# AnnaUshnova/tinyrenderder

Hardware: AMD Instinct MI355X
Metric: triangles/sec (+ Mpixels/sec) at 4096x4096; achieved HBM GB/s vs peak (higher is better)
Workload: dtype f64

## Files before the change

tinyrenderder_amd/csrc/kernels_bin.hip:

```cpp
#include <hip/hip_runtime.h>
#include <algorithm>
#include "trgl_device.h"
#include "launch.h"
#include "device_util.h"

namespace {

__device__ __forceinline__ double dmin3(double a, double b, double c) { double m = a; if (b < m) m = b; if (c < m) m = c; return m; }
__device__ __forceinline__ double dmax3(double a, double b, double c) { double m = a; if (m < b) m = b; if (m < c) m = c; return m; }
using trgl_dev::dot4; using trgl_dev::wave_incl_scan; using trgl_dev::block_excl_scan;

__device__ __forceinline__ int wave_min_i(int v) {
    for (int o = 32; o; o >>= 1) { int t = __shfl_xor(v, o); v = t < v ? t : v; }
    return v;
}
__device__ __forceinline__ int wave_max_i(int v) {
    for (int o = 32; o; o >>= 1) { int t = __shfl_xor(v, o); v = t > v ? t : v; }
    return v;
}

__device__ __forceinline__ uint32_t tile_block_mask(uint32_t tx, uint32_t ty, uint32_t qx0, uint32_t qy0, uint32_t qx1, uint32_t qy1) {
    const uint32_t c0 = qx0 > 4 * tx ? qx0 - 4 * tx : 0u, c1 = qx1 < 4 * tx + 3 ? qx1 - 4 * tx : 3u;
    const uint32_t r0 = qy0 > 4 * ty ? qy0 - 4 * ty : 0u, r1 = qy1 < 4 * ty + 3 ? qy1 - 4 * ty : 3u;
    return (((2u << c1) - (1u << c0)) & 0xfu) * 0x1111u & ((0xffffu >> (12 - 4 * r1)) & (0xffffu << (4 * r0)));
// ... 1 lines not shown
template <class Put>
__device__ __forceinline__ void block_pairs(const FrameParams& fp, int tiles_x, uint32_t i, uint32_t c, uint2 tb, uint32_t o, Put put) {
    constexpr uint32_t SMALL = 8;
    if (c && c <= SMALL) {
        const uint32_t qx0 = tb.x & 0x1fff, qy0 = (tb.x >> 16) & 0x1fff, qx1 = tb.y & 0x1fff, qy1 = (tb.y >> 16) & 0x1fff;
        const uint32_t iz = i | ((((tb.x >> 13) & 7u) | (((tb.y >> 13) & 7u) << 3) | ((tb.y >> 29) << 6)) << 25);
        const uint32_t tx0 = qx0 >> 2, ty0 = qy0 >> 2, tx1 = qx1 >> 2;
        uint32_t tx = tx0, row = 0;
        uint32_t ty = fp.il_tiles ? (uint32_t)il_nth_owned_from(fp, (int)ty0, 0) : ty0;
        for (uint32_t k = 0; k < c; ++k) {
            put(o + k, ty * tiles_x + tx, iz, tile_block_mask(tx, ty, qx0, qy0, qx1, qy1));
            if (++tx > tx1) { tx = tx0; ++row; ty = fp.il_tiles ? (uint32_t)il_nth_owned_from(fp, (int)ty0, (int)row) : ty0 + row; }
        }
    }
    unsigned long long big = __ballot(c > SMALL);
    const int lane = threadIdx.x & 63;
    while (big) {
        int src = __ffsll((long long)big) - 1;
        big &= big - 1;
        uint32_t cc = __shfl(c, src), oo = __shfl(o, src), ii = __shfl(i, src);
        uint32_t bx = __shfl(tb.x, src), by = __shfl(tb.y, src);
        const uint32_t qx0 = bx & 0x1fff, qy0 = (bx >> 16) & 0x1fff, qx1 = by & 0x1fff, qy1 = (by >> 16) & 0x1fff;
        ii |= (((bx >> 13) & 7u) | (((by >> 13) & 7u) << 3) | ((by >> 29) << 6)) << 25;
        uint32_t tx0 = qx0 >> 2, ty0 = qy0 >> 2, tx1 = qx1 >> 2;
        uint32_t wdt = tx1 - tx0 + 1;
        for (uint32_t k = lane; k < cc; k += 64) {
            uint32_t ty = fp.il_tiles ? (uint32_t)il_nth_owned_from(fp, (int)ty0, (int)(k / wdt)) : ty0 + k / wdt, tx = tx0 + k % wdt;
            put(oo + k, ty * tiles_x + tx, ii, tile_block_mask(tx, ty, qx0, qy0, qx1, qy1));
        }
    }
}

constexpr uint32_t SEG_MAX = 4096, SEG_MAX_GROUP = 16;

constexpr int SETUP_THREADS = 256;

__global__ __launch_bounds__(SETUP_THREADS) void k_setup(FrameParams fp, DrawDesc d, DrawDesc* __restrict__ draws_out, int draw_idx,
                                                         TriRec* __restrict__ recs, TriW* __restrict__ recs_w, uint32_t* __restrict__ cnt,
                                                         uint2* __restrict__ tilebox, DevStats* __restrict__ stats,
                                                         uint32_t* __restrict__ blk_sums, uint32_t blk_base,
                                                         uint32_t* __restrict__ seg_k, uint32_t* __restrict__ seg_v, uint32_t seg_S) {
    __shared__ __attribute__((aligned(16))) double s_buf[SETUP_THREADS * 16];
    if (blockIdx.x == 0 && threadIdx.x == 0) draws_out[draw_idx] = d;
    const uint32_t b0 = blockIdx.x * SETUP_THREADS;
    const uint32_t nb = min((uint32_t)SETUP_THREADS, d.n - b0);
    const uint32_t tid = threadIdx.x;
    const uint32_t i = b0 + tid;
    const bool in_range = tid < nb;

    const double* src = d.clip + (size_t)b0 * 12;
    if ((reinterpret_cast<uintptr_t>(src) & 15) == 0) {
        const double2* s2 = reinterpret_cast<const double2*>(src);
        double2* l2 = reinterpret_cast<double2*>(s_buf);
        typedef double f64x2 __attribute__((ext_vector_type(2)));
        for (uint32_t k = tid; k < nb * 6; k += SETUP_THREADS)
            *reinterpret_cast<f64x2*>(&l2[k]) = __builtin_nontemporal_load(reinterpret_cast<const f64x2*>(&s2[k]));
    } else {
        for (uint32_t k = tid; k < nb * 12; k += SETUP_THREADS) s_buf[k] = src[k];
    }
    __syncthreads();
    double v[12];
#pragma unroll
    for (int k = 0; k < 12; ++k) v[k] = in_range ? s_buf[tid * 12 + k] : 0.0;
    __syncthreads();

    int bx0 = INT_MAX, by0 = INT_MAX, bx1 = INT_MIN, by1 = INT_MIN;
    uint32_t ntiles = 0;
    bool large = false;
    uint2 tb = make_uint2(0, 0);
    TriRec r;
    {
        uint4* z4 = reinterpret_cast<uint4*>(&r);
#pragma unroll
        for (int k = 0; k < 8; ++k) z4[k] = make_uint4(0, 0, 0, 0);
// ... 97 lines not shown
        uint4* l4 = reinterpret_cast<uint4*>(s_buf);
        const uint4* r4 = reinterpret_cast<const uint4*>(&r);
#pragma unroll
        for (int c = 0; c < 8; ++c) l4[tid * 8 + (c ^ (tid & 7))] = r4[c];
        const unsigned long long keep = __ballot(ntiles != 0);
        __builtin_amdgcn_wave_barrier();
        uint4* dst = reinterpret_cast<uint4*>(recs + d.first + b0 + wbase);
#pragma unroll
        for (int it = 0; it < 8; ++it) {
            const uint32_t k = lane + 64u * it, t = k >> 3, c = k & 7;
            if ((keep >> t) & 1ull) {
                typedef uint32_t u32x4 __attribute__((ext_vector_type(4)));
                __builtin_nontemporal_store(*reinterpret_cast<const u32x4*>(&l4[(wbase + t) * 8 + (c ^ (t & 7))]), reinterpret_cast<u32x4*>(&dst[k]));
            }
        }
    }
    {
        const unsigned long long lit = __ballot(ntiles != 0 && r.ruz == 0.0);
        if (lit && lane == 0) atomicAdd(&stats->literal_tris, (unsigned long long)__popcll(lit));
        const unsigned long long lrg = __ballot(large);
        if (lrg && lane == 0) atomicAdd(&stats->large_tris, (unsigned long long)__popcll(lrg));
    }
    int wx0 = wave_min_i(bx0), wy0 = wave_min_i(by0), wx1 = wave_max_i(bx1), wy1 = wave_max_i(by1);
    if ((threadIdx.x & 63) == 0 && wx0 != INT_MAX) {
        if (wx0 < __builtin_nontemporal_load(&stats->min_x)) atomicMin(&stats->min_x, wx0);
        if (wy0 < __builtin_nontemporal_load(&stats->min_y)) atomicMin(&stats->min_y, wy0);
        if (wx1 > __builtin_nontemporal_load(&stats->max_x)) atomicMax(&stats->max_x, wx1);
        if (wy1 > __builtin_nontemporal_load(&stats->max_y)) atomicMax(&stats->max_y, wy1);
    }
    uint32_t tot;
    const uint32_t off = block_excl_scan(ntiles, reinterpret_cast<uint32_t*>(s_buf), &tot);
    if (tid == 0) blk_sums[blk_base + blockIdx.x] = tot;
    if (seg_S && tot && tot <= seg_S) {
        __syncthreads();
        uint32_t* const s_k = reinterpret_cast<uint32_t*>(s_buf);
        uint32_t* const s_v = s_k + SEG_MAX;
        block_pairs(fp, fp.tiles_x, d.first + i, ntiles, tb, off, [&](uint32_t j, uint32_t key, uint32_t iz, uint32_t m) { s_k[j] = key | (m << 16); s_v[j] = iz; });
        __syncthreads();
        uint4* const kq = reinterpret_cast<uint4*>(seg_k + (size_t)(blk_base + blockIdx.x) * seg_S);
        uint4* const vq = reinterpret_cast<uint4*>(seg_v + (size_t)(blk_base + blockIdx.x) * seg_S);
        for (uint32_t q = tid; 4 * q < tot; q += SETUP_THREADS) {
            kq[q] = *reinterpret_cast<const uint4*>(s_k + 4 * q);
            vq[q] = *reinterpret_cast<const uint4*>(s_v + 4 * q);
        }
    }
}

constexpr int EXPAND_CHUNK = 16;

constexpr int SPINE_THREADS = 1024;
__global__ __launch_bounds__(SPINE_THREADS) void k_chunk_spine(const uint32_t* __restrict__ blk_sums, uint32_t nblk,
                                                               uint32_t* __restrict__ chunk_off,
                                                               unsigned long long* __restrict__ total64, unsigned long long* __restrict__ host_copy,
                                                               uint4* __restrict__ bounds16, uint32_t n_half16,
                                                               uint32_t seg_S, uint32_t seg_G, uint32_t seg_chunk,
                                                               uint32_t* __restrict__ seg_flag, uint32_t* __restrict__ seg_flag_host) {
    __shared__ unsigned long long s_wave[SPINE_THREADS / 64];
    int seg_bad = seg_S == 0;
    if (seg_S && seg_G != EXPAND_CHUNK) {
        for (uint32_t g = threadIdx.x; (uint64_t)g * seg_G < nblk; g += SPINE_THREADS) {
            uint32_t t[EXPAND_CHUNK];
#pragma unroll
            for (uint32_t k = 0; k < EXPAND_CHUNK; ++k) { const uint32_t q = g * seg_G + k; t[k] = (k < seg_G && q < nblk) ? blk_sums[q] : 0u; }
            unsigned long long sum = 0;
#pragma unroll
            for (uint32_t k = 0; k < EXPAND_CHUNK; ++k) sum += t[k];
            seg_bad |= sum > seg_chunk;
        }
    }
    const uint32_t blk_max = seg_S ? seg_S : ~0u;
    const unsigned long long grp_max = (seg_S && seg_G == EXPAND_CHUNK) ? seg_chunk : ~0ull;
    for (uint32_t k = threadIdx.x; k < 2 * n_half16; k += SPINE_THREADS) bounds16[k] = k < n_half16 ? make_uint4(~0u, ~0u, ~0u, ~0u) : make_uint4(0, 0, 0, 0);
    const uint32_t nchunks = (nblk + EXPAND_CHUNK - 1) / EXPAND_CHUNK;
    const int lane = threadIdx.x & 63, w = threadIdx.x >> 6;
    unsigned long long running = 0;
    for (uint32_t start = 0; start < nchunks; start += SPINE_THREADS) {
        const uint32_t c = start + threadIdx.x;
        unsigned long long v = 0;
        if (c < nchunks) {
            const uint32_t q0 = c * EXPAND_CHUNK;
            if (q0 + EXPAND_CHUNK <= nblk) {
                const uint4* p4 = reinterpret_cast<const uint4*>(blk_sums + q0);
#pragma unroll
                for (int k = 0; k < EXPAND_CHUNK / 4; ++k) {
                    const uint4 t = p4[k]; v += (unsigned long long)t.x + t.y + t.z + t.w;
                    seg_bad |= max(max(t.x, t.y), max(t.z, t.w)) > blk_max;
                }
            } else {
                for (uint32_t q = q0; q < nblk; ++q) { const uint32_t t = blk_sums[q]; v += t; seg_bad |= t > blk_max; }
// ... 70 lines not shown
                    if (j >= sh && j < end) { kq[j] = s_k[j]; vq[j] = s_v[j]; if (WIDE) mq[j] = s_m[j]; }
            }
        }
    }
}

constexpr int RADIX_ROUNDS = 16;
constexpr int RADIX_WAVE_CHUNK = RADIX_ROUNDS * 64;
constexpr uint32_t RADIX_BIG_CAP = 4u << 20;
constexpr int RADIX_MAX_BITS = 8;

__global__ __launch_bounds__(256) void k_radix_hist(const uint32_t* __restrict__ keys, const unsigned long long* __restrict__ pairs_total,
                                                    uint32_t cap, int shift, int bits, uint32_t chunk,
                                                    uint32_t nblocks, uint32_t* __restrict__ hist, const uint32_t* __restrict__ skip) {
    __shared__ uint32_t s_cnt[1 << RADIX_MAX_BITS];
    const unsigned long long P64 = *pairs_total;
    const uint32_t P = (P64 > cap || (skip && *skip)) ? 0u : (uint32_t)P64;
    const uint32_t nb = 1u << bits, mask = nb - 1;
    for (uint32_t b = threadIdx.x; b < nb; b += 256) s_cnt[b] = 0;
    __syncthreads();
    const uint64_t beg = (uint64_t)blockIdx.x * chunk;
    uint64_t end = beg + chunk; if (end > P) end = P;
    for (uint64_t p = beg + 4u * threadIdx.x; p < end; p += 1024) {
        const uint4 q = *reinterpret_cast<const uint4*>(keys + p);
        const uint32_t k[4] = { q.x, q.y, q.z, q.w };
#pragma unroll
        for (int j = 0; j < 4; ++j) if (p + j < end) atomicAdd(&s_cnt[(k[j] >> shift) & mask], 1u);
    }
    __syncthreads();
    for (uint32_t b = threadIdx.x; b < nb; b += 256) hist[(size_t)b * nblocks + blockIdx.x] = s_cnt[b];
}

struct SegIn { const uint32_t* blk_sums; const uint32_t* flag; uint32_t nsetup, S, G; };

__global__ __launch_bounds__(256) void k_radix_hist_seg(const uint32_t* __restrict__ seg_k, SegIn seg, const unsigned long long* __restrict__ pairs_total,
                                                        uint32_t cap, int shift, int bits, uint32_t nblocks, uint32_t* __restrict__ hist) {
    __shared__ uint32_t s_cnt[1 << RADIX_MAX_BITS];
    const bool live = *seg.flag == 0 && *pairs_total <= cap;
    const uint32_t nb = 1u << bits, mask = nb - 1;
    for (uint32_t b = threadIdx.x; b < nb; b += 256) s_cnt[b] = 0;
    __syncthreads();
    const uint32_t w = threadIdx.x >> 6, lane = threadIdx.x & 63;
    if (live) {
        static_assert(SEG_MAX_GROUP == 16, "four waves of four segments");
        auto count4 = [&](const uint4 q, uint32_t p, uint32_t n) {
            const uint32_t k[4] = { q.x, q.y, q.z, q.w };
#pragma unroll
            for (int j = 0; j < 4; ++j) if (p + j < n) atomicAdd(&s_cnt[(k[j] >> shift) & mask], 1u);
        };
        uint32_t n[4]; const uint32_t* keys[4]; uint4 q[4][2];
#pragma unroll
        for (int j = 0; j < 4; ++j) {
            const uint32_t sg = w + 4 * j, b = blockIdx.x * seg.G + sg;
            const bool has = sg < seg.G && b < seg.nsetup;
            n[j] = has ? min(seg.blk_sums[b], seg.S) : 0u;
            keys[j] = seg_k + (size_t)(has ? b : 0u) * seg.S;
        }
#pragma unroll
        for (int j = 0; j < 4; ++j)
#pragma unroll
            for (int it = 0; it < 2; ++it) {
                const uint32_t p = 4 * lane + 256 * it;
                q[j][it] = p < n[j] ? *reinterpret_cast<const uint4*>(keys[j] + p) : make_uint4(0, 0, 0, 0);
            }
#pragma unroll
        for (int j = 0; j < 4; ++j) {
#pragma unroll
            for (int it = 0; it < 2; ++it) count4(q[j][it], 4 * lane + 256 * it, n[j]);
            for (uint32_t p = 512 + 4 * lane; p < n[j]; p += 256) count4(*reinterpret_cast<const uint4*>(keys[j] + p), p, n[j]);
        }
    }
    __syncthreads();
    for (uint32_t b = threadIdx.x; b < nb; b += 256) hist[(size_t)b * nblocks + blockIdx.x] = s_cnt[b];
}

constexpr int ROWSCAN_THREADS = 1024, ROWSCAN_PER = 8;
__global__ __launch_bounds__(ROWSCAN_THREADS) void k_radix_scan_rows(uint32_t* __restrict__ hist, uint32_t nblocks, uint32_t* __restrict__ totals) {
    __shared__ uint32_t s_wave[ROWSCAN_THREADS / 64];
    uint32_t* row = hist + (size_t)blockIdx.x * nblocks;
    const int lane = threadIdx.x & 63, w = threadIdx.x >> 6;
    uint32_t running = 0;
    for (uint32_t start = 0; start < nblocks; start += ROWSCAN_THREADS * ROWSCAN_PER) {
        const uint32_t base = start + threadIdx.x * ROWSCAN_PER;
        uint32_t v[ROWSCAN_PER], sum = 0;
#pragma unroll
        for (int k = 0; k < ROWSCAN_PER; ++k) { v[k] = (base + k < nblocks) ? row[base + k] : 0; sum += v[k]; }
        uint32_t inc = sum;
        for (int o = 1; o < 64; o <<= 1) { const uint32_t t = __shfl_up(inc, o); if (lane >= o) inc += t; }
        if (lane == 63) s_wave[w] = inc;
        __syncthreads();
        uint32_t wbase = 0, tot = 0;
#pragma unroll
        for (int k = 0; k < ROWSCAN_THREADS / 64; ++k) { const uint32_t t = s_wave[k]; if (k < w) wbase += t; tot += t; }
        uint32_t run = running + wbase + inc - sum;
#pragma unroll
        for (int k = 0; k < ROWSCAN_PER; ++k) { if (base + k < nblocks) row[base + k] = run; run += v[k]; }
        running += tot;
        __syncthreads();
    }
    if (threadIdx.x == 0) totals[blockIdx.x] = running;
}

template <int R, int N, class F>
__device__ __forceinline__ void rounds_below(uint32_t part, F& f) {
    if constexpr (R < N) {
        if ((uint32_t)(R * 64) < part) { f(R); rounds_below<R + 1, N>(part, f); }
    }
// ... 174 lines not shown
    constexpr uint32_t KEY_MASK = WIDE ? 0xffffffffu : 0xffffu;
    for (uint32_t i = threadIdx.x; i < n_chunk; i += RADIX_THREADS) {
        const uint32_t word = s_key[i];
        const uint32_t dgt = (word >> shift) & mask;
        const uint32_t dst = s_gbase[dgt] + (i - s_start[dgt]);
        vals_out[dst] = s_val[i];
        if (!LAST) {
            keys_out[dst] = word;
            if (WIDE) msk_out[dst] = s_msk[i];
        } else {
            msk_out[dst] = WIDE ? s_msk[i] : (uint16_t)(word >> 16);
            const uint32_t key = word & KEY_MASK;
            if (i == 0 || (s_key[i - 1] & KEY_MASK) != key) atomicMin(&tile_start[key], dst);
            if (i + 1 == n_chunk || (s_key[i + 1] & KEY_MASK) != key) atomicMax(&tile_end[key], dst + 1);
        }
    }
    if (!more) break;
    chunk = next; cur = nxt;
    __syncthreads();
    }
}

}

namespace trgl {

uint32_t setup_num_blocks(uint32_t n) { return (n + SETUP_THREADS - 1) / SETUP_THREADS; }

void launch_setup(hipStream_t s, const FrameParams& fp, const DrawDesc& draw, DrawDesc* draws_dev, int draw_idx, uint32_t n,
                  TriRec* recs, TriW* recs_w, uint32_t* cnt, uint2* tilebox, DevStats* stats, uint32_t* blk_sums, uint32_t blk_base,
                  const SegLayout* seg) {
    if (!n) return;
    hipLaunchKernelGGL(k_setup, dim3(setup_num_blocks(n)), dim3(SETUP_THREADS), 0, s, fp, draw, draws_dev, draw_idx, recs, recs_w, cnt, tilebox,
                       stats, blk_sums, blk_base, seg ? seg->keys : nullptr, seg ? seg->vals : nullptr, seg ? seg->S : 0u);
}

void launch_chunk_spine(hipStream_t s, const uint32_t* blk_sums, uint32_t nblk, uint32_t* chunk_off, unsigned long long* total64, unsigned long long* host_copy,
                        uint32_t* tile_bounds, size_t half_words, uint32_t seg_S, uint32_t seg_G, uint32_t seg_chunk, uint32_t* seg_flag,
                        uint32_t* seg_flag_host) {
    hipLaunchKernelGGL(k_chunk_spine, dim3(1), dim3(SPINE_THREADS), 0, s, blk_sums, nblk, chunk_off, total64, host_copy, (uint4*)tile_bounds,
                       (uint32_t)(half_words / 4), seg_S, seg_G, seg_chunk, seg_flag, seg_flag_host);
}

void launch_expand(hipStream_t s, const FrameParams& fp, uint32_t first, uint32_t n, int tiles_x, const uint32_t* cnt, const uint32_t* blk_sums,
                   const uint32_t* chunk_off, uint32_t blk_base, const uint2* tilebox, uint32_t* keys, bool wide, uint32_t* vals, uint16_t* bmask,
                   const unsigned long long* pairs_total, uint32_t cap) {
    if (!n) return;
    if (wide)
        hipLaunchKernelGGL(k_expand<true>, dim3(setup_num_blocks(n)), dim3(SETUP_THREADS), 0, s, fp, first, n, tiles_x, cnt, blk_sums, chunk_off,
                           blk_base, tilebox, keys, vals, bmask, pairs_total, cap);
    else
        hipLaunchKernelGGL(k_expand<false>, dim3(setup_num_blocks(n)), dim3(SETUP_THREADS), 0, s, fp, first, n, tiles_x, cnt, blk_sums, chunk_off,
                           blk_base, tilebox, keys, vals, bmask, pairs_total, cap);
}

static uint32_t radix_waves(uint32_t cap) { return cap >= RADIX_BIG_CAP ? 8u : 4u; }
uint32_t radix_chunk(uint32_t cap) { return radix_waves(cap) * RADIX_WAVE_CHUNK; }
uint32_t radix_num_workers(uint32_t cap) { const uint64_t chunk = radix_chunk(cap); return (uint32_t)((cap + chunk - 1) / chunk); }
uint32_t seg_num_groups(const SegLayout& seg) { return (seg.nsetup + seg.G - 1) / seg.G; }
bool seg_layout_ok(const SegLayout& seg) { return seg.S >= 4 && seg.S <= SEG_MAX && seg.S % 4 == 0 && seg.G >= 1 && seg.G <= SEG_MAX_GROUP; }

template <int WAVES, bool WIDE, bool LAST, bool SEG>
static uint32_t scatter_grid(uint32_t chunks, uint32_t max_blocks) {
    thread_local int for_dev = -1;
    thread_local uint32_t resident = 0;
    int dev = 0;
    if (hipGetDevice(&dev) != hipSuccess) dev = 0;
    if (dev != for_dev) {
        int per_cu = 0, cus = 0;
        if (hipOccupancyMaxActiveBlocksPerMultiprocessor(&per_cu, k_radix_scatter<WAVES, WIDE, LAST, SEG>, WAVES * 64, 0) != hipSuccess || per_cu < 1) per_cu = 1;
        if (hipDeviceGetAttribute(&cus, hipDeviceAttributeMultiprocessorCount, dev) != hipSuccess || cus < 1) cus = 1;
        resident = (uint32_t)per_cu * (uint32_t)cus;
        for_dev = dev;
    }
    uint32_t g = std::min(chunks, resident);
    if (max_blocks) g = std::min(g, max_blocks);
    return std::max(g, 1u);
}

template <int WAVES, bool WIDE, bool LAST>
static uint32_t radix_pass_t(hipStream_t s, const RadixPass& ps, const unsigned long long* pairs_total, uint32_t cap, uint32_t* hist, uint32_t* scan_tmp,
                             const uint32_t* skip, uint32_t max_blocks) {
    const uint32_t nblk = radix_num_workers(cap), grid = scatter_grid<WAVES, WIDE, LAST, false>(nblk, max_blocks);
    hipLaunchKernelGGL(k_radix_hist, dim3(nblk), dim3(256), 0, s, ps.keys_in, pairs_total, cap, ps.shift, ps.bits, (uint32_t)(WAVES * RADIX_WAVE_CHUNK),
                       nblk, hist, skip);
    hipLaunchKernelGGL(k_radix_scan_rows, dim3(1u << ps.bits), dim3(ROWSCAN_THREADS), 0, s, hist, nblk, scan_tmp);
    hipLaunchKernelGGL((k_radix_scatter<WAVES, WIDE, LAST, false>), dim3(grid), dim3(WAVES * 64), 0, s, ps.keys_in, ps.vals_in, ps.msk_in, pairs_total, cap,
                       ps.shift, ps.bits, nblk, hist, scan_tmp, ps.keys_out, ps.vals_out, ps.msk_out, ps.tile_start, ps.tile_end, SegIn{ nullptr, skip, 0, 0, 0 });
    return grid;
}
template <int WAVES, bool LAST>
static uint32_t radix_pass_seg(hipStream_t s, const RadixPass& ps, const SegLayout& sl, const unsigned long long* pairs_total, uint32_t cap, uint32_t* hist,
                               uint32_t* scan_tmp, uint32_t max_blocks) {
    const uint32_t nblk = seg_num_groups(sl), grid = scatter_grid<WAVES, false, LAST, true>(nblk, max_blocks);
    const SegIn seg{ sl.blk_sums, sl.flag, sl.nsetup, sl.S, sl.G };
    hipLaunchKernelGGL(k_radix_hist_seg, dim3(nblk), dim3(256), 0, s, sl.keys, seg, pairs_total, cap, ps.shift, ps.bits, nblk, hist);
    hipLaunchKernelGGL(k_radix_scan_rows, dim3(1u << ps.bits), dim3(ROWSCAN_THREADS), 0, s, hist, nblk, scan_tmp);
    hipLaunchKernelGGL((k_radix_scatter<WAVES, false, LAST, true>), dim3(grid), dim3(WAVES * 64), 0, s, sl.keys, sl.vals, ps.msk_in, pairs_total, cap,
                       ps.shift, ps.bits, nblk, hist, scan_tmp, ps.keys_out, ps.vals_out, ps.msk_out, ps.tile_start, ps.tile_end, seg);
    return grid;
}

template <int WAVES>
static uint32_t radix_pass_w(hipStream_t s, const RadixPass& ps, bool wide, bool last, const unsigned long long* pairs_total, uint32_t cap,
                             uint32_t* hist, uint32_t* scan_tmp, const SegLayout* seg, const uint32_t* skip, uint32_t mb) {
    if (seg) return last ? radix_pass_seg<WAVES, true>(s, ps, *seg, pairs_total, cap, hist, scan_tmp, mb) : radix_pass_seg<WAVES, false>(s, ps, *seg, pairs_total, cap, hist, scan_tmp, mb);
    if (wide) return last ? radix_pass_t<WAVES, true, true>(s, ps, pairs_total, cap, hist, scan_tmp, skip, mb) : radix_pass_t<WAVES, true, false>(s, ps, pairs_total, cap, hist, scan_tmp, skip, mb);
    return last ? radix_pass_t<WAVES, false, true>(s, ps, pairs_total, cap, hist, scan_tmp, skip, mb) : radix_pass_t<WAVES, false, false>(s, ps, pairs_total, cap, hist, scan_tmp, skip, mb);
}

uint32_t launch_radix_pass(hipStream_t s, const RadixPass& ps, bool wide, bool last, const unsigned long long* pairs_total, uint32_t cap,
                           uint32_t* hist, uint32_t* scan_tmp, const SegLayout* seg, const uint32_t* skip, uint32_t max_blocks) {
    if (!cap || (seg && (wide || !seg->nsetup))) return 0;
    if (radix_waves(cap) == 8) return radix_pass_w<8>(s, ps, wide, last, pairs_total, cap, hist, scan_tmp, seg, skip, max_blocks);
    return radix_pass_w<4>(s, ps, wide, last, pairs_total, cap, hist, scan_tmp, seg, skip, max_blocks);
}

}
```

tinyrenderder_amd/csrc/launch.h:

```cpp
#pragma once
#include <hip/hip_runtime.h>
#include "trgl_device.h"
#include "clip_core.h"
#include "work_items.h"

namespace trgl {

struct SegLayout { uint32_t* keys; uint32_t* vals; const uint32_t* blk_sums; const uint32_t* flag; uint32_t nsetup, S, G; };
bool seg_layout_ok(const SegLayout& seg);
uint32_t seg_num_groups(const SegLayout& seg);

uint32_t setup_num_blocks(uint32_t n);
void launch_setup(hipStream_t s, const FrameParams& fp, const DrawDesc& draw, DrawDesc* draws_dev, int draw_idx, uint32_t n,
                  TriRec* recs, TriW* recs_w, uint32_t* cnt, uint2* tilebox, DevStats* stats, uint32_t* blk_sums, uint32_t blk_base,
                  const SegLayout* seg);
void launch_chunk_spine(hipStream_t s, const uint32_t* blk_sums, uint32_t nblk, uint32_t* chunk_off, unsigned long long* total64, unsigned long long* host_copy,
                        uint32_t* tile_bounds, size_t half_words, uint32_t seg_S, uint32_t seg_G, uint32_t seg_chunk, uint32_t* seg_flag,
                        uint32_t* seg_flag_host);


void launch_expand(hipStream_t s, const FrameParams& fp, uint32_t first, uint32_t n, int tiles_x, const uint32_t* cnt, const uint32_t* blk_sums,
                   const uint32_t* chunk_off, uint32_t blk_base, const uint2* tilebox, uint32_t* keys, bool wide, uint32_t* vals, uint16_t* bmask,
                   const unsigned long long* pairs_total, uint32_t cap);

uint32_t radix_num_workers(uint32_t cap);
uint32_t radix_chunk(uint32_t cap);
struct RadixPass {
    const uint32_t* keys_in; const uint32_t* vals_in; const uint16_t* msk_in;
    uint32_t* keys_out; uint32_t* vals_out; uint16_t* msk_out;
    uint32_t* tile_start; uint32_t* tile_end;
    int shift, bits;
};
uint32_t launch_radix_pass(hipStream_t s, const RadixPass& ps, bool wide, bool last, const unsigned long long* pairs_total, uint32_t cap,
                           uint32_t* hist, uint32_t* scan_tmp, const SegLayout* seg = nullptr, const uint32_t* skip = nullptr,
                           uint32_t max_blocks = 0);

uint32_t owned_tiles(const FrameParams& fp);
uint32_t raster_max_items(const FrameParams& fp);
void launch_make_items(hipStream_t s, const FrameParams& fp, int tiles, const uint32_t* tile_start, const uint32_t* tile_end, uint4* items,
                       uint32_t* n_items, TriRec* recs);
void launch_fold_stats(hipStream_t s, DevStats* stats, uint32_t* n_items, const unsigned long long* item_stats);
struct UserShade { hipFunction_t fn; int kind; };
void launch_raster(hipStream_t s, const FrameParams& fp, int kind, bool all_well_scaled, const TriRec* recs, const TriW* recs_w,
                   const uint32_t* vals, const uint16_t* bmask,
                   const uint32_t* tile_start, const uint32_t* tile_end, const DrawDesc* draws,
                   const DevTexture* tex, DevStats* stats, uint32_t max_items, uint4* items,
                   uint32_t* n_items, unsigned long long* item_stats, bool builtin_shade, const UserShade* user, int n_user,
                   hipFunction_t user_raster,
                   hipEvent_t ev_before = nullptr, hipEvent_t ev_after = nullptr);

void launch_vertex_stage(hipStream_t s, const double mv[16], const double proj[16], const double* vertices, int stride,
// ... 87 lines not shown
```

tinyrenderder_amd/csrc/trgl_api.cpp:

```cpp
#include <algorithm>
#include <cstring>

#include "trgl_ctx.h"
#include "user_shaders.h"

static size_t pair_capacity(size_t need) {
    const size_t ncap = (headroom(need) + 3) & ~size_t(3);
    return ncap > 0xffffe000ull ? 0xffffe000ull : ncap;
}

int trgl::fail(trgl_ctx* c, int code, const std::string& msg) { if (c) c->err = msg; else set_global_error(msg); return code; }

static int reset_dev_stats(trgl_ctx* c) {
    DevStats s;
    s.fragments = 0;
    s.zmin_key = zkey(std::numeric_limits<double>::infinity());
    s.zmax_key = zkey(-std::numeric_limits<double>::infinity());
    s.min_x = INT32_MAX; s.min_y = INT32_MAX; s.max_x = INT32_MIN; s.max_y = INT32_MIN;
    s.pairs_total = 0; s.literal_tris = 0; s.large_tris = 0;
    s.zero_pos_key = s.zero_neg_key = TRGL_ZERO_KEY_EMPTY;
    s.zero_locked = 0; s.zero_sign = 0;
    for (int k = 0; k < 16; ++k) s.dbg[k] = 0;
    *c->stats_pinned = s;
    HIPCHK(c, hipMemcpyAsync(c->stats_dev.p, c->stats_pinned, sizeof(DevStats), hipMemcpyHostToDevice, c->stream));
// ... 215 lines not shown
        DrawDesc d; std::memset(&d, 0, sizeof(d));
        d.n = (uint32_t)m; d.first = (uint32_t)c->queued_tris; d.kind = kind; d.K = K;
        if (u) d.u = *u; else { d.u.tex_diffuse = d.u.tex_normal = d.u.tex_specular = -1; }
        d.clip = dclip + done * 12;
        d.vary = dvary ? dvary + done * K : nullptr;
        d.colors = dcol ? dcol + done : nullptr;
        c->draws.push_back(d);
        c->queued_tris += m;
        done += m;
    }
    return TRGL_OK;
}

static int resolve_events(trgl_ctx* c) {
    if (!c->events_pending) return TRGL_OK;
    HIPCHK(c, hipEventSynchronize(c->ev[3]));
    float ms;
    HIPCHK(c, hipEventElapsedTime(&ms, c->ev[0], c->ev[1])); c->phase_ms[TRGL_PHASE_SETUP] += ms;
    HIPCHK(c, hipEventElapsedTime(&ms, c->ev[1], c->ev[2])); c->phase_ms[TRGL_PHASE_BIN] += ms;
    HIPCHK(c, hipEventElapsedTime(&ms, c->ev[2], c->ev[3])); c->phase_ms[TRGL_PHASE_RASTER] += ms;
    HIPCHK(c, hipEventElapsedTime(&ms, c->ev[0], c->ev[3])); c->phase_ms[TRGL_PHASE_TOTAL] += ms;
    HIPCHK(c, hipEventElapsedTime(&ms, c->ev[4], c->ev[5])); c->phase_ms[TRGL_PHASE_RASTER_KERNEL] += ms;
    c->flushes_timed++;
    c->events_pending = false;
    return TRGL_OK;
}

int trgl_flush(trgl_ctx* c) {
    CHKCTX(c);
    int r = trgl_flush_begin(c);
    return r ? r : trgl_flush_end(c);
}

static int queue_binning(trgl_ctx* c, const FrameParams& fp, uint32_t cap, int* cur_out, const SegLayout* seg) {
    hipStream_t s = c->stream;
    const size_t ntiles = (size_t)c->tiles_x * c->tiles_y;
    const unsigned long long* pairs_dev = &c->stats_dev.p->pairs_total;
    int r;
    uint32_t blk_base = 0;
    const bool wide = ntiles > 65536;
    for (auto& d : c->draws) {
        if (seg) break;
        launch_expand(s, fp, d.first, d.n, c->tiles_x, c->cnt.p, c->blk_sums.p, c->chunk_off.p, blk_base, c->tilebox.p, c->keys[0].p, wide, c->vals[0].p,
                      c->bmask[0].p, pairs_dev, cap);
        blk_base += setup_num_blocks(d.n);
    }
    int key_bits = 1; while ((size_t(1) << key_bits) < ntiles) ++key_bits;
    int passes = (key_bits + 7) / 8;
    int bits_per = (key_bits + passes - 1) / passes;
    size_t hist_need = ((size_t)std::max(radix_num_workers(cap), seg ? seg_num_groups(*seg) : 0u) << bits_per) + 16;
    if ((r = c->hist.grow(c, hist_need))) return r;
    if ((r = c->scan_tmp.grow(c, 256 + 16))) return r;
    int cur = 0;
    for (int ps = 0; ps < passes; ++ps) {
        const RadixPass rp{ c->keys[cur].p, c->vals[cur].p, c->bmask[cur].p, c->keys[cur ^ 1].p, c->vals[cur ^ 1].p, c->bmask[cur ^ 1].p,
                            c->tile_start.p, c->tile_end(), ps * bits_per, bits_per };
        const uint32_t grid = launch_radix_pass(s, rp, wide, ps == passes - 1, pairs_dev, cap, c->hist.p, c->scan_tmp.p, ps == 0 ? seg : nullptr,
                                                (seg && ps > 0) ? seg->flag : nullptr, c->radix_max_blocks);
        if (ps == 0) c->radix_used[0] = grid;
        if (ps == passes - 1) c->radix_used[1] = grid;
        cur ^= 1;
    }
    *cur_out = cur;
    return TRGL_OK;
}

static int grow_pairs(trgl_ctx* c, size_t need) {
    const size_t ncap = pair_capacity(need);
    int r;
    for (int k = 0; k < 2; ++k)
        if ((r = c->keys[k].grow(c, need, ncap)) || (r = c->vals[k].grow(c, need, ncap)) || (r = c->bmask[k].grow(c, need, ncap))) return r;
    return TRGL_OK;
}

static bool seg_sizes(double avg, uint32_t chunk, uint32_t* S, uint32_t* G) {
    if (avg < 1.0) avg = 1.0;
    const uint64_t s = ((uint64_t)(avg * 1.5) + 128 + 63) & ~uint64_t(63);
    uint64_t g = (uint64_t)(0.9 * chunk / avg);
    if (g > 16) g = 16;
    if (s > 4096 || g < 2) return false;
    *S = (uint32_t)s; *G = (uint32_t)g;
    return true;
}
constexpr uint64_t SEG_MAX_BYTES = uint64_t(1) << 30;

static int settle_binning(trgl_ctx* c, bool may_grow) {
    PendingRaster& rp = c->rp;
    if (!rp.N || rp.settled) return TRGL_OK;
    HIPCHK(c, hipEventSynchronize(c->ev_pairs));
    const unsigned long long P64 = c->stats_pinned->pairs_total;
    if (P64 > 0xffffe000ull) return TRGL_OK;
    const bool bad = *c->seg_flag_pinned != 0, over = P64 > rp.cap, fell = rp.direct && bad;
    if (over && !may_grow) return TRGL_OK;
    int r;
    if (over || fell) {
        if (over && (r = grow_pairs(c, (size_t)P64))) return r;
        if ((r = queue_binning(c, rp.fp, (uint32_t)c->keys[0].cap, &rp.cur, fell ? nullptr : (rp.direct ? &rp.seg : nullptr)))) return r;
        rp.cap = (uint32_t)c->keys[0].cap;
        if (c->profiling) HIPCHK(c, hipEventRecord(c->ev[2], c->stream));
    }
    if (c->bin_mode == 0) { if (fell) c->seg_hold = true; else if (!rp.direct && !bad) c->seg_hold = false; }
    rp.fell_back = fell; rp.settled = true;
    return TRGL_OK;
}

static FrameParams frame_params(const trgl_ctx* c) {
    FrameParams fp; std::memset(&fp, 0, sizeof(fp));
    fp.fb = c->fb.p; fp.zb = c->zb.p; fp.W = c->W; fp.H = c->H; fp.bpp = c->bpp;
    fp.tiles_x = c->tiles_x; fp.tiles_y = c->tiles_y;
    fp.strip_y0 = c->strip_y0; fp.strip_y1 = c->strip_y1;
    fp.strip_ty0 = c->strip_y0 / TRGL_TILE;
    fp.strip_ty1 = (c->strip_y1 + TRGL_TILE - 1) / TRGL_TILE;
    if (c->strip_y1 <= c->strip_y0) fp.strip_ty1 = fp.strip_ty0;
    fp.il_tiles = c->il_tiles; fp.il_world = c->il_world; fp.il_rank = c->il_rank;
    fp.init_from_clear = c->clear_pending ? 1 : 0;
    fp.n_tris = (uint32_t)c->queued_tris;
    fp.clear_color = c->clear_color; fp.clear_z = c->clear_z;
    std::memcpy(fp.vp, c->vp, sizeof(fp.vp));
    return fp;
}

int trgl_flush_begin(trgl_ctx* c) {
    CHKCTX(c);
    if (c->rp.active) return TRGL_OK;
    if (c->draws.empty() && !c->clear_pending) return TRGL_OK;
    int r;
    if ((r = resolve_events(c))) return r;
    c->snap.valid = false;
    const uint64_t N = c->queued_tris;
    hipStream_t s = c->stream;
// ... 3 lines not shown
    for (auto& d : c->draws) if (d.kind != flush_kind) flush_kind = -1;
    bool builtin_shade = false;
    uint32_t user_kinds = 0;
    for (auto& d : c->draws) {
        if (d.kind == TRGL_SHADER_PHONG || d.kind == TRGL_SHADER_EYE) builtin_shade = true;
        if (d.kind >= TRGL_SHADER_USER_FIRST && !discarding_kind(c, d.kind)) user_kinds |= 1u << (d.kind - TRGL_SHADER_USER_FIRST);
        if (discarding_kind(c, d.kind) && d.kind != flush_kind) return fail(c, TRGL_E_STATE, "flush: a kind that may discard shares a flush with another kind");
    }
    if (builtin_shade || user_kinds) {
        if ((r = c->idbuf.grow(c, (size_t)c->W * c->H))) return r;
        fp.idbuf = c->idbuf.p;
    }

    if (c->profiling) HIPCHK(c, hipEventRecord(c->ev[0], s));
    uint32_t cap = 0;
    int cur = 0;
    if (N) {
        const size_t tcap = headroom(N);
        if ((r = c->recs.grow(c, N + 1, tcap)) || (r = c->recs_w.grow(c, N + 1, tcap)) || (r = c->cnt.grow(c, N + 1, tcap)) ||
            (r = c->tilebox.grow(c, N + 1, tcap))) return r;
        if (c->keys[0].cap == 0 && (r = grow_pairs(c, (size_t)2 * N + 4096))) return r;
        uint32_t nblk = 0;
        for (auto& d : c->draws) nblk += setup_num_blocks(d.n);
        if ((r = c->blk_sums.grow(c, (size_t)nblk + 16))) return r;
        if ((r = c->chunk_off.grow(c, (size_t)nblk / 16 + 16))) return r;
        cap = (uint32_t)c->keys[0].cap;
        uint32_t S = 0, G = 0;
        bool direct = false;
        if ((size_t)c->tiles_x * c->tiles_y <= 65536) {
            if (c->bin_mode == 2) { S = c->bin_S; G = c->bin_G; direct = true; }
            else if (c->bin_mode == 0 && seg_sizes(c->rule_nblk ? (double)c->rule_pairs / (double)c->rule_nblk : 512.0, radix_chunk(cap), &S, &G))
                direct = !c->seg_hold && (uint64_t)nblk * S * 8 <= SEG_MAX_BYTES;
        }
        if (direct && ((r = c->seg_keys.grow(c, (size_t)nblk * S + 4)) || (r = c->seg_vals.grow(c, (size_t)nblk * S + 4)))) return r;
        const SegLayout seg{ c->seg_keys.p, c->seg_vals.p, c->blk_sums.p, c->seg_flag.p, nblk, S, G };
        c->rp.direct = direct; c->rp.seg = seg; c->rp.nblk = nblk;
        {
            uint32_t blk_base = 0;
            for (size_t i = 0; i < c->draws.size(); ++i) {
                launch_setup(s, fp, c->draws[i], c->draws_dev.p, (int)i, c->draws[i].n, c->recs.p, c->recs_w.p, c->cnt.p, c->tilebox.p, c->stats_dev.p,
                             c->blk_sums.p, blk_base, direct ? &seg : nullptr);
                blk_base += setup_num_blocks(c->draws[i].n);
            }
        }
        if (c->profiling) HIPCHK(c, hipEventRecord(c->ev[1], s));
        launch_chunk_spine(s, c->blk_sums.p, nblk, c->chunk_off.p, &c->stats_dev.p->pairs_total, &c->stats_pinned->pairs_total,
                           c->tile_start.p, c->bounds_half(), S, G, radix_chunk(cap), c->seg_flag.p, c->seg_flag_pinned);
        HIPCHK(c, hipEventRecord(c->ev_pairs, s));
        if ((r = queue_binning(c, fp, cap, &cur, direct ? &seg : nullptr))) return r;
    } else {
        c->rp.direct = false; c->rp.nblk = 0; c->rp.seg = SegLayout{};
        if (c->profiling) HIPCHK(c, hipEventRecord(c->ev[1], s));
        HIPCHK(c, hipMemsetAsync(c->tile_start.p, 0, c->bounds_half() * 8, s));
    }
    if (c->profiling) HIPCHK(c, hipEventRecord(c->ev[2], s));
    c->rp.active = true; c->rp.fp = fp; c->rp.flush_kind = flush_kind; c->rp.cap = cap; c->rp.cur = cur; c->rp.N = N;
    c->rp.builtin_shade = builtin_shade; c->rp.user_kinds = user_kinds;
    c->rp.settled = false; c->rp.fell_back = false;
    return TRGL_OK;
}

int trgl_flush_end(trgl_ctx* c) {
    CHKCTX(c);
    if (!c->rp.active) return TRGL_OK;
    c->rp.active = false;
    int r;
    hipStream_t s = c->stream;
    FrameParams fp = c->rp.fp;
    const int flush_kind = c->rp.flush_kind;
    int cur = c->rp.cur;
    const uint64_t N = c->rp.N;
    uint32_t P = 0;
    if (N) {
        HIPCHK(c, hipEventSynchronize(c->ev_pairs));
        const unsigned long long P64 = c->stats_pinned->pairs_total;
        if (P64 > 0xffffe000ull) {
            c->draws.clear(); c->queued_tris = 0;
            return fail(c, TRGL_E_UNSUPPORTED, "flush: more than 2^32 triangle-tile pairs; submit in smaller batches");
        }
        P = (uint32_t)P64;
        if ((r = settle_binning(c, true))) return r;
        cur = c->rp.cur;
// ... 207 lines not shown
```

tinyrenderder_amd/csrc/trgl_ctx.h:

```cpp
#pragma once
#include <hip/hip_runtime.h>

#include <limits>
#include <string>
#include <vector>

#include "../../include/trgl.h"
#include "launch.h"
#include "trgl_device.h"

namespace trgl {
struct StageChunk { char* base; size_t cap, used; };

inline size_t headroom(size_t need) { return need + need / 4 + 1024; }
template <class T> struct DevBuf {
    T* p = nullptr;
    size_t cap = 0;
    DevBuf() = default;
    DevBuf(const DevBuf&) = delete;
    ~DevBuf() { if (p) (void)hipFree(p); }
    int alloc(trgl_ctx* c, size_t n);
    int grow(trgl_ctx* c, size_t need, size_t ncap) { return need <= cap ? TRGL_OK : alloc(c, ncap); }
    int grow(trgl_ctx* c, size_t need) { return grow(c, need, headroom(need)); }
    int release(trgl_ctx* c);
// ... 20 lines not shown
    uint32_t clear_color = 0xff000000u;
    double clear_z = std::numeric_limits<double>::infinity();
    int strip_y0 = 0, strip_y1 = 0;
    int il_tiles = 0, il_world = 1, il_rank = 0;

    DevTexture tex_host[TRGL_MAX_TEXTURES];
    DevBuf<DevTexture> tex_dev;

    std::vector<DrawDesc> draws;
    uint64_t queued_tris = 0;
    std::vector<StageChunk> stage;
    int stage_hold = 0;

    DevBuf<TriRec> recs; DevBuf<TriW> recs_w; DevBuf<uint32_t> cnt; DevBuf<uint2> tilebox;
    PendingRaster rp;
    hipEvent_t ev_pairs = nullptr;
    DevBuf<uint32_t> idbuf;
    DevBuf<BoundsPartial> bounds_scratch;
    DevBuf<uint8_t> mesh_scratch;
    DevBuf<double> zsnap[TRGL_MAX_Z_SNAPSHOTS];
    DevBuf<float> blur_weights; DevBuf<uint8_t> blur_tmp; int blur_radius = 0;
    float* blur_w_pinned = nullptr; size_t blur_w_pinned_cap = 0; hipEvent_t ev_blur_w = nullptr;
    DevBuf<uint32_t> clip_scratch;
    DevBuf<uint8_t> shadow_tmp;
    DevBuf<double> occl_levels, occl_boxes; DevBuf<uint8_t> occl_codes;
    DevBuf<uint32_t> inst_scratch, inst_list; DevBuf<double> inst_mv;
    DevBuf<uint8_t> order_scratch;
    DevBuf<uint8_t> pp_out;
    DevBuf<uint32_t> blk_sums;
    DevBuf<uint32_t> chunk_off;
    DevBuf<uint32_t> keys[2], vals[2]; DevBuf<uint16_t> bmask[2];
    DevBuf<uint32_t> hist, scan_tmp;
    DevBuf<uint32_t> seg_keys, seg_vals, seg_flag;
    uint32_t* seg_flag_pinned = nullptr;
    int bin_mode = 0; uint32_t bin_S = 0, bin_G = 0;
    bool seg_hold = false;
    uint32_t radix_max_blocks = 0, radix_used[2] = { 0, 0 };
    uint64_t rule_pairs = 0, rule_nblk = 0;
    DevBuf<uint32_t> tile_start;
    DevBuf<uint4> items; DevBuf<uint32_t> n_items;
    DevBuf<unsigned long long> item_stats;
    DevBuf<DrawDesc> draws_dev;
    DevBuf<DevStats> stats_dev;
    DevStats* stats_pinned = nullptr;

    uint64_t triangles_total = 0;
    Snapshot snap;

    bool profiling = false, events_pending = false;
    hipEvent_t ev[6] = { nullptr, nullptr, nullptr, nullptr, nullptr, nullptr };
    double phase_ms[TRGL_NUM_PHASES] = { 0, 0, 0, 0, 0 };
    uint64_t flushes_timed = 0;

    std::vector<UserKind> user;
    std::vector<UserVertex> vertex;

    std::string err;

    size_t bounds_half() const { return ((size_t)tiles_x * tiles_y + 3) & ~size_t(3); }
    uint32_t* tile_end() const { return tile_start.p + bounds_half(); }
};

#define HIPCHK(ctx, expr)                                                                      \
    do {                                                                                       \
        hipError_t e_ = (expr);                                                                \
        if (e_ != hipSuccess) {                                                                \
// ... 51 lines not shown
```

Baseline: 4.277 billion.

## Compute segment radix histograms in setup and fold them inside the spine kernel

```diff
diff --git a/tinyrenderder_amd/csrc/kernels_bin.hip b/tinyrenderder_amd/csrc/kernels_bin.hip
--- a/tinyrenderder_amd/csrc/kernels_bin.hip
+++ b/tinyrenderder_amd/csrc/kernels_bin.hip
@@ -57,6 +57,7 @@
 }
 
 constexpr uint32_t SEG_MAX = 4096, SEG_MAX_GROUP = 16;
+constexpr uint32_t SEG_DIGITS = 256;
 
 constexpr int SETUP_THREADS = 256;
 
@@ -64,7 +65,8 @@
                                                          TriRec* __restrict__ recs, TriW* __restrict__ recs_w, uint32_t* __restrict__ cnt,
                                                          uint2* __restrict__ tilebox, DevStats* __restrict__ stats,
                                                          uint32_t* __restrict__ blk_sums, uint32_t blk_base,
-                                                         uint32_t* __restrict__ seg_k, uint32_t* __restrict__ seg_v, uint32_t seg_S) {
+                                                         uint32_t* __restrict__ seg_k, uint32_t* __restrict__ seg_v, uint32_t seg_S,
+                                                         uint16_t* __restrict__ seg_hist, uint32_t seg_bits) {
     __shared__ __attribute__((aligned(16))) double s_buf[SETUP_THREADS * 16];
     if (blockIdx.x == 0 && threadIdx.x == 0) draws_out[draw_idx] = d;
     const uint32_t b0 = blockIdx.x * SETUP_THREADS;
@@ -228,10 +230,18 @@
     const uint32_t off = block_excl_scan(ntiles, reinterpret_cast<uint32_t*>(s_buf), &tot);
     if (tid == 0) blk_sums[blk_base + blockIdx.x] = tot;
     if (seg_S && tot && tot <= seg_S) {
-        __syncthreads();
         uint32_t* const s_k = reinterpret_cast<uint32_t*>(s_buf);
         uint32_t* const s_v = s_k + SEG_MAX;
-        block_pairs(fp, fp.tiles_x, d.first + i, ntiles, tb, off, [&](uint32_t j, uint32_t key, uint32_t iz, uint32_t m) { s_k[j] = key | (m << 16); s_v[j] = iz; });
+        const bool behind = tot <= SEG_MAX - SEG_DIGITS;
+        uint32_t* const s_h = behind ? s_k + (SEG_MAX - SEG_DIGITS) : s_v;
+        const uint32_t dmask = (1u << seg_bits) - 1u;
+        static_assert(SETUP_THREADS == SEG_DIGITS, "a counter per thread");
+        if (behind) s_h[tid] = 0;
+        __syncthreads();
+        block_pairs(fp, fp.tiles_x, d.first + i, ntiles, tb, off, [&](uint32_t j, uint32_t key, uint32_t iz, uint32_t m) {
+            s_k[j] = key | (m << 16); s_v[j] = iz;
+            if (behind) atomicAdd(&s_h[key & dmask], 1u);
+        });
         __syncthreads();
         uint4* const kq = reinterpret_cast<uint4*>(seg_k + (size_t)(blk_base + blockIdx.x) * seg_S);
         uint4* const vq = reinterpret_cast<uint4*>(seg_v + (size_t)(blk_base + blockIdx.x) * seg_S);
@@ -239,18 +249,69 @@
             kq[q] = *reinterpret_cast<const uint4*>(s_k + 4 * q);
             vq[q] = *reinterpret_cast<const uint4*>(s_v + 4 * q);
         }
+        if (!behind) {
+            __syncthreads();
+            s_h[tid] = 0;
+            __syncthreads();
+            for (uint32_t j = tid; j < tot; j += SETUP_THREADS) atomicAdd(&s_h[s_k[j] & dmask], 1u);
+            __syncthreads();
+        }
+        uint32_t* const row = reinterpret_cast<uint32_t*>(seg_hist + ((size_t)(blk_base + blockIdx.x) << seg_bits));
+        if (2 * tid <= dmask) row[tid] = s_h[2 * tid] | (s_h[2 * tid + 1] << 16);
     }
 }
 
 constexpr int EXPAND_CHUNK = 16;
 
 constexpr int SPINE_THREADS = 1024;
+
+struct SegFold { const uint16_t* seg_hist; uint32_t* table; int bits; };
+constexpr uint32_t FOLD_GROUPS = SPINE_THREADS / 64;
+__device__ __forceinline__ void seg_fold_block(const uint32_t fb, const SegFold f, const uint32_t* __restrict__ blk_sums, const uint32_t nsetup,
+                                               const uint32_t S, const uint32_t G) {
+    __shared__ uint32_t s_sum[FOLD_GROUPS][SEG_DIGITS + 1];
+    const uint32_t w = threadIdx.x >> 6, lane = threadIdx.x & 63;
+    const uint32_t nb = 1u << f.bits, ngroups = (nsetup + G - 1) / G;
+    const uint32_t g = fb * FOLD_GROUPS + w;
+    uint32_t sum[4] = { 0, 0, 0, 0 };
+    if (g < ngroups) {
+        const uint32_t bl = g * G + (lane & (SEG_MAX_GROUP - 1));
+        const uint32_t nl = ((lane & (SEG_MAX_GROUP - 1)) < G && bl < nsetup) ? blk_sums[bl] : 0u;
+        uint2 q[SEG_MAX_GROUP];
+#pragma unroll
+        for (uint32_t k = 0; k < SEG_MAX_GROUP; ++k) {
+            const uint32_t b = g * G + k;
+            q[k] = make_uint2(0, 0);
+            if (k < G && b < nsetup && 4 * lane < nb) {
+                const uint16_t* const row = f.seg_hist + ((size_t)b << f.bits) + 4 * lane;
+                if (nb >= 4) q[k] = *reinterpret_cast<const uint2*>(row);
+                else q[k].x = *reinterpret_cast<const uint32_t*>(row);
+            }
+        }
+#pragma unroll
+        for (uint32_t k = 0; k < SEG_MAX_GROUP; ++k) {
+            const uint32_t n = __shfl(nl, k);
+            if (n && n <= S) { sum[0] += q[k].x & 0xffffu; sum[1] += q[k].x >> 16; sum[2] += q[k].y & 0xffffu; sum[3] += q[k].y >> 16; }
+        }
+    }
+#pragma unroll
+    for (uint32_t j = 0; j < 4; ++j) s_sum[w][4 * lane + j] = sum[j];
+    __syncthreads();
+    const uint32_t g0 = fb * FOLD_GROUPS;
+    for (uint32_t t = threadIdx.x; t < nb * FOLD_GROUPS; t += SPINE_THREADS) {
+        const uint32_t d = t / FOLD_GROUPS, k = t % FOLD_GROUPS;
+        if (g0 + k < ngroups) f.table[(size_t)d * ngroups + g0 + k] = s_sum[k][d];
+    }
+}
+
 __global__ __launch_bounds__(SPINE_THREADS) void k_chunk_spine(const uint32_t* __restrict__ blk_sums, uint32_t nblk,
                                                                uint32_t* __restrict__ chunk_off,
                                                                unsigned long long* __restrict__ total64, unsigned long long* __restrict__ host_copy,
                                                                uint4* __restrict__ bounds16, uint32_t n_half16,
                                                                uint32_t seg_S, uint32_t seg_G, uint32_t seg_chunk,
-                                                               uint32_t* __restrict__ seg_flag, uint32_t* __restrict__ seg_flag_host) {
+                                                               uint32_t* __restrict__ seg_flag, uint32_t* __restrict__ seg_flag_host,
+                                                               SegFold fold, uint32_t spine_blocks) {
+    if (blockIdx.x >= spine_blocks) { seg_fold_block(blockIdx.x - spine_blocks, fold, blk_sums, nblk, seg_S, seg_G); return; }
     __shared__ unsigned long long s_wave[SPINE_THREADS / 64];
     int seg_bad = seg_S == 0;
     if (seg_S && seg_G != EXPAND_CHUNK) {
@@ -387,47 +448,6 @@
 }
 
 struct SegIn { const uint32_t* blk_sums; const uint32_t* flag; uint32_t nsetup, S, G; };
-
-__global__ __launch_bounds__(256) void k_radix_hist_seg(const uint32_t* __restrict__ seg_k, SegIn seg, const unsigned long long* __restrict__ pairs_total,
-                                                        uint32_t cap, int shift, int bits, uint32_t nblocks, uint32_t* __restrict__ hist) {
-    __shared__ uint32_t s_cnt[1 << RADIX_MAX_BITS];
-    const bool live = *seg.flag == 0 && *pairs_total <= cap;
-    const uint32_t nb = 1u << bits, mask = nb - 1;
-    for (uint32_t b = threadIdx.x; b < nb; b += 256) s_cnt[b] = 0;
-    __syncthreads();
-    const uint32_t w = threadIdx.x >> 6, lane = threadIdx.x & 63;
-    if (live) {
-        static_assert(SEG_MAX_GROUP == 16, "four waves of four segments");
-        auto count4 = [&](const uint4 q, uint32_t p, uint32_t n) {
-            const uint32_t k[4] = { q.x, q.y, q.z, q.w };
-#pragma unroll
-            for (int j = 0; j < 4; ++j) if (p + j < n) atomicAdd(&s_cnt[(k[j] >> shift) & mask], 1u);
-        };
-        uint32_t n[4]; const uint32_t* keys[4]; uint4 q[4][2];
-#pragma unroll
-        for (int j = 0; j < 4; ++j) {
-            const uint32_t sg = w + 4 * j, b = blockIdx.x * seg.G + sg;
-            const bool has = sg < seg.G && b < seg.nsetup;
-            n[j] = has ? min(seg.blk_sums[b], seg.S) : 0u;
-            keys[j] = seg_k + (size_t)(has ? b : 0u) * seg.S;
-        }
-#pragma unroll
-        for (int j = 0; j < 4; ++j)
-#pragma unroll
-            for (int it = 0; it < 2; ++it) {
-                const uint32_t p = 4 * lane + 256 * it;
-                q[j][it] = p < n[j] ? *reinterpret_cast<const uint4*>(keys[j] + p) : make_uint4(0, 0, 0, 0);
-            }
-#pragma unroll
-        for (int j = 0; j < 4; ++j) {
-#pragma unroll
-            for (int it = 0; it < 2; ++it) count4(q[j][it], 4 * lane + 256 * it, n[j]);
-            for (uint32_t p = 512 + 4 * lane; p < n[j]; p += 256) count4(*reinterpret_cast<const uint4*>(keys[j] + p), p, n[j]);
-        }
-    }
-    __syncthreads();
-    for (uint32_t b = threadIdx.x; b < nb; b += 256) hist[(size_t)b * nblocks + blockIdx.x] = s_cnt[b];
-}
 
 constexpr int ROWSCAN_THREADS = 1024, ROWSCAN_PER = 8;
 __global__ __launch_bounds__(ROWSCAN_THREADS) void k_radix_scan_rows(uint32_t* __restrict__ hist, uint32_t nblocks, uint32_t* __restrict__ totals) {
@@ -668,14 +688,25 @@
                   const SegLayout* seg) {
     if (!n) return;
     hipLaunchKernelGGL(k_setup, dim3(setup_num_blocks(n)), dim3(SETUP_THREADS), 0, s, fp, draw, draws_dev, draw_idx, recs, recs_w, cnt, tilebox,
-                       stats, blk_sums, blk_base, seg ? seg->keys : nullptr, seg ? seg->vals : nullptr, seg ? seg->S : 0u);
-}
+                       stats, blk_sums, blk_base, seg ? seg->keys : nullptr, seg ? seg->vals : nullptr, seg ? seg->S : 0u,
+                       seg ? seg->hist : nullptr, seg ? (uint32_t)seg->bits : 0u);
+}
+
+static uint32_t fold_num_blocks(const SegLayout& seg) { return (seg_num_groups(seg) + FOLD_GROUPS - 1) / FOLD_GROUPS; }
 
 void launch_chunk_spine(hipStream_t s, const uint32_t* blk_sums, uint32_t nblk, uint32_t* chunk_off, unsigned long long* total64, unsigned long long* host_copy,
                         uint32_t* tile_bounds, size_t half_words, uint32_t seg_S, uint32_t seg_G, uint32_t seg_chunk, uint32_t* seg_flag,
-                        uint32_t* seg_flag_host) {
-    hipLaunchKernelGGL(k_chunk_spine, dim3(1), dim3(SPINE_THREADS), 0, s, blk_sums, nblk, chunk_off, total64, host_copy, (uint4*)tile_bounds,
-                       (uint32_t)(half_words / 4), seg_S, seg_G, seg_chunk, seg_flag, seg_flag_host);
+                        uint32_t* seg_flag_host, const SegLayout* fold, uint32_t* table) {
+    const bool folds = fold && fold->nsetup;
+    hipLaunchKernelGGL(k_chunk_spine, dim3(1 + (folds ? fold_num_blocks(*fold) : 0u)), dim3(SPINE_THREADS), 0, s, blk_sums, nblk, chunk_off, total64,
+                       host_copy, (uint4*)tile_bounds, (uint32_t)(half_words / 4), seg_S, seg_G, seg_chunk, seg_flag, seg_flag_host,
+                       SegFold{ folds ? fold->hist : nullptr, table, folds ? fold->bits : 0 }, 1u);
+}
+
+void launch_seg_fold(hipStream_t s, const SegLayout& fold, uint32_t* table) {
+    if (!fold.nsetup) return;
+    hipLaunchKernelGGL(k_chunk_spine, dim3(fold_num_blocks(fold)), dim3(SPINE_THREADS), 0, s, fold.blk_sums, fold.nsetup, nullptr, nullptr, nullptr, nullptr,
+                       0u, fold.S, fold.G, 0u, nullptr, nullptr, SegFold{ fold.hist, table, fold.bits }, 0u);
 }
 
 void launch_expand(hipStream_t s, const FrameParams& fp, uint32_t first, uint32_t n, int tiles_x, const uint32_t* cnt, const uint32_t* blk_sums,
@@ -694,6 +725,7 @@
 uint32_t radix_chunk(uint32_t cap) { return radix_waves(cap) * RADIX_WAVE_CHUNK; }
 uint32_t radix_num_workers(uint32_t cap) { const uint64_t chunk = radix_chunk(cap); return (uint32_t)((cap + chunk - 1) / chunk); }
 uint32_t seg_num_groups(const SegLayout& seg) { return (seg.nsetup + seg.G - 1) / seg.G; }
+static_assert(SEG_DIGITS == 1u << RADIX_MAX_BITS, "a counter per digit of a pass");
 bool seg_layout_ok(const SegLayout& seg) { return seg.S >= 4 && seg.S <= SEG_MAX && seg.S % 4 == 0 && seg.G >= 1 && seg.G <= SEG_MAX_GROUP; }
 
 template <int WAVES, bool WIDE, bool LAST, bool SEG>
@@ -730,7 +762,6 @@
                                uint32_t* scan_tmp, uint32_t max_blocks) {
     const uint32_t nblk = seg_num_groups(sl), grid = scatter_grid<WAVES, false, LAST, true>(nblk, max_blocks);
     const SegIn seg{ sl.blk_sums, sl.flag, sl.nsetup, sl.S, sl.G };
-    hipLaunchKernelGGL(k_radix_hist_seg, dim3(nblk), dim3(256), 0, s, sl.keys, seg, pairs_total, cap, ps.shift, ps.bits, nblk, hist);
     hipLaunchKernelGGL(k_radix_scan_rows, dim3(1u << ps.bits), dim3(ROWSCAN_THREADS), 0, s, hist, nblk, scan_tmp);
     hipLaunchKernelGGL((k_radix_scatter<WAVES, false, LAST, true>), dim3(grid), dim3(WAVES * 64), 0, s, sl.keys, sl.vals, ps.msk_in, pairs_total, cap,
                        ps.shift, ps.bits, nblk, hist, scan_tmp, ps.keys_out, ps.vals_out, ps.msk_out, ps.tile_start, ps.tile_end, seg);
diff --git a/tinyrenderder_amd/csrc/launch.h b/tinyrenderder_amd/csrc/launch.h
--- a/tinyrenderder_amd/csrc/launch.h
+++ b/tinyrenderder_amd/csrc/launch.h
@@ -6,7 +6,7 @@
 
 namespace trgl {
 
-struct SegLayout { uint32_t* keys; uint32_t* vals; const uint32_t* blk_sums; const uint32_t* flag; uint32_t nsetup, S, G; };
+struct SegLayout { uint32_t* keys; uint32_t* vals; const uint32_t* blk_sums; const uint32_t* flag; uint32_t nsetup, S, G; uint16_t* hist; int bits; };
 bool seg_layout_ok(const SegLayout& seg);
 uint32_t seg_num_groups(const SegLayout& seg);
 
@@ -16,7 +16,8 @@
                   const SegLayout* seg);
 void launch_chunk_spine(hipStream_t s, const uint32_t* blk_sums, uint32_t nblk, uint32_t* chunk_off, unsigned long long* total64, unsigned long long* host_copy,
                         uint32_t* tile_bounds, size_t half_words, uint32_t seg_S, uint32_t seg_G, uint32_t seg_chunk, uint32_t* seg_flag,
-                        uint32_t* seg_flag_host);
+                        uint32_t* seg_flag_host, const SegLayout* fold, uint32_t* table);
+void launch_seg_fold(hipStream_t s, const SegLayout& fold, uint32_t* table);
 
 
 void launch_expand(hipStream_t s, const FrameParams& fp, uint32_t first, uint32_t n, int tiles_x, const uint32_t* cnt, const uint32_t* blk_sums,
diff --git a/tinyrenderder_amd/csrc/trgl_api.cpp b/tinyrenderder_amd/csrc/trgl_api.cpp
--- a/tinyrenderder_amd/csrc/trgl_api.cpp
+++ b/tinyrenderder_amd/csrc/trgl_api.cpp
@@ -271,7 +271,20 @@
     return r ? r : trgl_flush_end(c);
 }
 
-static int queue_binning(trgl_ctx* c, const FrameParams& fp, uint32_t cap, int* cur_out, const SegLayout* seg) {
+struct RadixPlan { int passes, bits_per; };
+static RadixPlan radix_plan(const trgl_ctx* c) {
+    const size_t ntiles = (size_t)c->tiles_x * c->tiles_y;
+    int key_bits = 1; while ((size_t(1) << key_bits) < ntiles) ++key_bits;
+    const int passes = (key_bits + 7) / 8;
+    return RadixPlan{ passes, (key_bits + passes - 1) / passes };
+}
+static int grow_hist(trgl_ctx* c, uint32_t cap, const SegLayout* seg) {
+    int r;
+    if ((r = c->hist.grow(c, ((size_t)std::max(radix_num_workers(cap), seg ? seg_num_groups(*seg) : 0u) << radix_plan(c).bits_per) + 16))) return r;
+    return c->scan_tmp.grow(c, 256 + 16);
+}
+
+static int queue_binning(trgl_ctx* c, const FrameParams& fp, uint32_t cap, int* cur_out, const SegLayout* seg, bool refold) {
     hipStream_t s = c->stream;
     const size_t ntiles = (size_t)c->tiles_x * c->tiles_y;
     const unsigned long long* pairs_dev = &c->stats_dev.p->pairs_total;
@@ -284,12 +297,9 @@
                       c->bmask[0].p, pairs_dev, cap);
         blk_base += setup_num_blocks(d.n);
     }
-    int key_bits = 1; while ((size_t(1) << key_bits) < ntiles) ++key_bits;
-    int passes = (key_bits + 7) / 8;
-    int bits_per = (key_bits + passes - 1) / passes;
-    size_t hist_need = ((size_t)std::max(radix_num_workers(cap), seg ? seg_num_groups(*seg) : 0u) << bits_per) + 16;
-    if ((r = c->hist.grow(c, hist_need))) return r;
-    if ((r = c->scan_tmp.grow(c, 256 + 16))) return r;
+    const int passes = radix_plan(c).passes, bits_per = radix_plan(c).bits_per;
+    if ((r = grow_hist(c, cap, seg))) return r;
+    if (seg && refold) launch_seg_fold(s, *seg, c->hist.p);
     int cur = 0;
     for (int ps = 0; ps < passes; ++ps) {
         const RadixPass rp{ c->keys[cur].p, c->vals[cur].p, c->bmask[cur].p, c->keys[cur ^ 1].p, c->vals[cur ^ 1].p, c->bmask[cur ^ 1].p,
@@ -334,7 +344,7 @@
     int r;
     if (over || fell) {
         if (over && (r = grow_pairs(c, (size_t)P64))) return r;
-        if ((r = queue_binning(c, rp.fp, (uint32_t)c->keys[0].cap, &rp.cur, fell ? nullptr : (rp.direct ? &rp.seg : nullptr)))) return r;
+        if ((r = queue_binning(c, rp.fp, (uint32_t)c->keys[0].cap, &rp.cur, fell ? nullptr : (rp.direct ? &rp.seg : nullptr), true))) return r;
         rp.cap = (uint32_t)c->keys[0].cap;
         if (c->profiling) HIPCHK(c, hipEventRecord(c->ev[2], c->stream));
     }
@@ -404,8 +414,11 @@
             else if (c->bin_mode == 0 && seg_sizes(c->rule_nblk ? (double)c->rule_pairs / (double)c->rule_nblk : 512.0, radix_chunk(cap), &S, &G))
                 direct = !c->seg_hold && (uint64_t)nblk * S * 8 <= SEG_MAX_BYTES;
         }
-        if (direct && ((r = c->seg_keys.grow(c, (size_t)nblk * S + 4)) || (r = c->seg_vals.grow(c, (size_t)nblk * S + 4)))) return r;
-        const SegLayout seg{ c->seg_keys.p, c->seg_vals.p, c->blk_sums.p, c->seg_flag.p, nblk, S, G };
+        const int seg_bits = radix_plan(c).bits_per;
+        if (direct && ((r = c->seg_keys.grow(c, (size_t)nblk * S + 4)) || (r = c->seg_vals.grow(c, (size_t)nblk * S + 4)) ||
+                       (r = c->seg_hist.grow(c, ((size_t)nblk << seg_bits) + 4)))) return r;
+        const SegLayout seg{ c->seg_keys.p, c->seg_vals.p, c->blk_sums.p, c->seg_flag.p, nblk, S, G, c->seg_hist.p, seg_bits };
+        if (direct && (r = grow_hist(c, cap, &seg))) return r;
         c->rp.direct = direct; c->rp.seg = seg; c->rp.nblk = nblk;
         {
             uint32_t blk_base = 0;
@@ -417,9 +430,10 @@
         }
         if (c->profiling) HIPCHK(c, hipEventRecord(c->ev[1], s));
         launch_chunk_spine(s, c->blk_sums.p, nblk, c->chunk_off.p, &c->stats_dev.p->pairs_total, &c->stats_pinned->pairs_total,
-                           c->tile_start.p, c->bounds_half(), S, G, radix_chunk(cap), c->seg_flag.p, c->seg_flag_pinned);
+                           c->tile_start.p, c->bounds_half(), S, G, radix_chunk(cap), c->seg_flag.p, c->seg_flag_pinned,
+                           direct ? &seg : nullptr, c->hist.p);
         HIPCHK(c, hipEventRecord(c->ev_pairs, s));
-        if ((r = queue_binning(c, fp, cap, &cur, direct ? &seg : nullptr))) return r;
+        if ((r = queue_binning(c, fp, cap, &cur, direct ? &seg : nullptr, false))) return r;
     } else {
         c->rp.direct = false; c->rp.nblk = 0; c->rp.seg = SegLayout{};
         if (c->profiling) HIPCHK(c, hipEventRecord(c->ev[1], s));
diff --git a/tinyrenderder_amd/csrc/trgl_ctx.h b/tinyrenderder_amd/csrc/trgl_ctx.h
--- a/tinyrenderder_amd/csrc/trgl_ctx.h
+++ b/tinyrenderder_amd/csrc/trgl_ctx.h
@@ -76,6 +76,7 @@
     DevBuf<uint32_t> keys[2], vals[2]; DevBuf<uint16_t> bmask[2];
     DevBuf<uint32_t> hist, scan_tmp;
     DevBuf<uint32_t> seg_keys, seg_vals, seg_flag;
+    DevBuf<uint16_t> seg_hist;
     uint32_t* seg_flag_pinned = nullptr;
     int bin_mode = 0; uint32_t bin_S = 0, bin_G = 0;
     bool seg_hold = false;
```

Measured after the change: 4.292 billion, median of 6. Within noise of the previous version (+0.4%).
